# Greketrotny/RayZath

Hardware: AMD Instinct MI355X
Metric: Mrays/s (path segments, primary+secondary) at 1920x1080 depth 8 (higher is better)
Workload: dtype f32; 1 GPU; Cornell box 1920x1080 depth 8; max_depth=8, triangles=16, instances=8, traversal=workgroup-binned, integrator=CPU kernel (parity-checked), pipeline=resident (one kernel per step)

## Files before the change

rayzath_amd/csrc/hiprz_api.hip:

```cpp
#include <hip/hip_runtime.h>

#include <algorithm>
#include <cmath>
#include <cstdio>
#include <cstdlib>
#include <cstring>
#include <string>
#include <vector>

#include "hiprz.h"
#include "hiprz_ctx.hpp"
#include "hiprz_device.hpp"

using namespace hiprz;


__global__ void __launch_bounds__(256) rz_order_keys_kernel(const uint32_t* cost, uint32_t* keys, uint32_t n) {
    const uint32_t i = blockIdx.x * 256u + threadIdx.x;
    if (i < n) keys[i] = 0x00FFFFFFu - (cost[i] < 0x00FFFFFFu ? cost[i] : 0x00FFFFFFu);
}

__global__ void rz_pass_update_kernel(uint32_t* pass) { *pass += 1u; }
__global__ void rz_pass_reset_kernel(uint32_t* pass) { *pass = 0u; }
__global__ void rz_pass_add_kernel(uint32_t* pass, uint32_t n) { *pass += n; }
// ... 93 lines not shown
                if (kind >= 4u) {
                    const bool of_a = kind < 6u;
                    WalkRay probe = q;
                    probe.far_ = RZ_FLT_MAX;
                    float t = 0.0f, u, v, det;
                    if (tri_hit(xyz(of_a ? ta[0] : tb[0]), xyz(of_a ? ta[1] : tb[1]), xyz(of_a ? ta[2] : tb[2]), probe, t, u, v, det)) {
                        if (kind & 1u) q.far_ = t;
                        else q.near_ = t;
                    }
                }
                const bool has_b = (h & 0xC00u) != 0u;
                WalkRay seq = q;
                uint32_t seq_tri = 0xFFFFFFFFu;
                float seq_b1 = 0.0f, seq_b2 = 0.0f;
                bool seq_external = false;
                {
                    float t, u, v, det;
                    if (tri_hit(xyz(ta[0]), xyz(ta[1]), xyz(ta[2]), seq, t, u, v, det)) {
                        seq.far_ = t;
                        seq_tri = 0u, seq_b1 = u, seq_b2 = v, seq_external = det > 0.0f;
                    }
                    if (has_b && tri_hit(xyz(tb[0]), xyz(tb[1]), xyz(tb[2]), seq, t, u, v, det)) {
                        seq.far_ = t;
                        seq_tri = 1u, seq_b1 = u, seq_b2 = v, seq_external = det > 0.0f;
                    }
                }
                LeafBest best;
                best.far_ = q.far_, best.triangle = 0xFFFFFFFFu, best.b1 = best.b2 = 0.0f, best.external = false;
                tri_pair_step(ta[0], ta[1], ta[2], has_b ? tb[0] : ta[0], has_b ? tb[1] : ta[1], has_b ? tb[2] : ta[2], 0u, has_b ? 1u : 0u, has_b, q, best);
                if (__float_as_uint(best.far_) != __float_as_uint(seq.far_) || best.triangle != seq_tri || __float_as_uint(best.b1) != __float_as_uint(seq_b1) ||
                    __float_as_uint(best.b2) != __float_as_uint(seq_b2) || best.external != seq_external)
                    bad += 1;
            }
        }
    }
    atomicAdd(&out[0], (unsigned long long)bad);
    atomicAdd(&out[1], (unsigned long long)tested);
    atomicAdd(&out[2], (unsigned long long)undecided);
}

namespace hiprz {
thread_local std::string g_create_error;
int fail(hiprz_ctx* ctx, int code, const std::string& msg) {
    if (ctx) ctx->error = msg;
    else g_create_error = msg;
    return code;
}
std::vector<KernelEntry>& kernel_table() {
    static std::vector<KernelEntry> table;
    return table;
}
void register_kernel(const void* stub, const char* name) { kernel_table().push_back(KernelEntry{stub, name}); }
int resolve_kernels(int device) {
    static std::vector<int> checked;
    for (int d : checked)
        if (d == device) return HIPRZ_OK;
    for (const KernelEntry& e : kernel_table()) {
        hipFuncAttributes attr;
        const hipError_t err = hipFuncGetAttributes(&attr, e.stub);
        if (err != hipSuccess) {
            (void)hipGetLastError();
            return fail(nullptr, HIPRZ_ERR_DEVICE, std::string("libhiprz.so is inconsistent: the loaded gfx950 code objects do not hold a kernel the host side can launch (") +
                                                       hipGetErrorString(err) + "): " + e.name + " — rebuild (make -C rayzath_amd/csrc; tools/check_kernels.py)");
        }
    }
    checked.push_back(device);
// ... 991 lines not shown
```

rayzath_amd/csrc/hiprz_device.hpp:

```cpp
#pragma once
#include <hip/hip_runtime.h>
#include <stdint.h>

#include "hiprz.h"
#include "hiprz_end.hpp"
#include "hiprz_lds.hpp"
#include "hiprz_shard.hpp"

#define RZ_DEV __device__ __forceinline__
#include "hiprz_flat_pick.hpp"
#include "hiprz_pair_pick.hpp"

namespace hiprz {

#ifndef RZ_FUSED_SHARED_RCP
#define RZ_FUSED_SHARED_RCP 0
#endif
#ifndef RZ_TRACE_SHARED_RCP
#define RZ_TRACE_SHARED_RCP 1
#endif
#ifndef RZ_BATCH_SHARED_RCP
#define RZ_BATCH_SHARED_RCP 1
#endif
#ifndef RZ_FLAT_PACKED_BOXES
#define RZ_FLAT_PACKED_BOXES 0
#endif
#ifndef RZ_FLAT_PAIR_TRIS
#define RZ_FLAT_PAIR_TRIS 1
#endif
#ifndef RZ_TRACE_MIN_WAVES
#define RZ_TRACE_MIN_WAVES 5
#endif
#define RZ_PI_F 3.14159265358979323846f
#define RZ_GUARD_LIMIT (1u << 26)
#ifndef RZ_WALK_GUARD
#define RZ_WALK_GUARD 0
#endif
#if RZ_WALK_GUARD
#define RZ_GUARD(counter) \
    if (++(counter) > RZ_GUARD_LIMIT) break
#else
#define RZ_GUARD(counter) (void)(counter)
#endif
#define RZ_FLT_MAX 3.402823466e+38f

#define RZ_SINF(x) sinf(x)
#define RZ_COSF(x) cosf(x)
#define RZ_SINCOSF(x, s, c) sincosf((x), &(s), &(c))
#define RZ_ACOSF(x) acosf(x)
#define RZ_ASINF(x) asinf(x)
#define RZ_ATAN2F(y, x) atan2f(y, x)
#define RZ_POWF(x, y) powf(x, y)
#define RZ_EXPF(x) expf(x)
#define RZ_LOGF(x) logf(x)

struct DScene {
    const float4* nodes;
    const uint32_t* tlas_order;
    const float4* tris;
    const float4* tri_attrs;
    const float4* instances;
    const int32_t* inst_materials;
    const float4* materials;
    const float4* textures;
    const uint8_t* texels;
    const float4* spot_lights;
    const float4* direct_lights;
    uint32_t n_instances;
    uint32_t tlas_root;
    uint32_t n_spot_lights;
    uint32_t n_direct_lights;
    uint32_t fast_div;
    uint32_t hot_bytes;
    const float4* hot;
    uint32_t off_nodes, off_tlas_order, off_instances, off_tris, off_tri_attrs, off_materials, off_inst_materials;
    uint32_t world_stack_entries;
    uint32_t mesh_stack_entries;
    float bounds_min[3];
    float bounds_scale[3];
    uint32_t top_count;
    const uint32_t* node_skip;
    uint32_t walk_k, walk_l;
    uint32_t walk_advance;
    uint32_t world_advance;
    uint32_t walk_h;
    const float4* nodes64;
    uint32_t shadow_variant;
    const float4* shadow_nodes64;
    const uint32_t* shadow_order;
    uint32_t shadow_root;
    uint32_t sort_variant;
};

RZ_DEV void repoint_hot(DScene& v, const unsigned char* base) {
    v.nodes = reinterpret_cast<const float4*>(base + v.off_nodes);
    v.tlas_order = reinterpret_cast<const uint32_t*>(base + v.off_tlas_order);
    v.instances = reinterpret_cast<const float4*>(base + v.off_instances);
    v.tris = reinterpret_cast<const float4*>(base + v.off_tris);
    v.tri_attrs = reinterpret_cast<const float4*>(base + v.off_tri_attrs);
    v.materials = reinterpret_cast<const float4*>(base + v.off_materials);
    v.inst_materials = reinterpret_cast<const int32_t*>(base + v.off_inst_materials);
}

struct DCamera {
    float position[3];
    float x_axis[3], y_axis[3], z_axis[3];
    uint32_t width, height;
    float tan_half_fov, aspect_ratio;
    float near_, far_;
    float focal_distance, aperture, exposure_time;
};

struct DConfig {
    uint32_t max_depth, spot_samples, direct_samples, seed;
    uint32_t flags;
};

struct DFrame {
    float4* st0;
    float4* st1;
    float2* st2;
    float4* accum;
    float4* hit0;
    uint32_t* hit1;
    float* depth;
    uint32_t* rgba8;
    const uint32_t* pass;
    unsigned long long* counters;
    uint32_t tiles_x;
    uint32_t rank, world;
    uint32_t n_local_tiles;
    uint32_t* sort_key;
    const uint32_t* perm;
    uint32_t xcd_swizzle;
    float4* nee;
// ... 333 lines not shown
    r = __builtin_elementwise_fma(nd, q, n);
    return __builtin_elementwise_fma(r, yy, q);
}
RZ_DEV void box_range_pairs(float4 b0, float4 b1, const WalkRayPairs& p, float& tmin, float& tmax) {
    const f2 tx = div_pairs(f2{b0.x, b0.y} - p.ox, p.ndx, p.yx);
    const f2 ty = div_pairs(f2{b0.z, b0.w} - p.oy, p.ndy, p.yy);
    const f2 tz = div_pairs(f2{b1.x, b1.y} - p.oz, p.ndz, p.yz);
    tmin = vmax3(vmin(tx.x, tx.y), vmin(ty.x, ty.y), vmin(tz.x, tz.y));
    tmax = vmin3(vmax(tx.x, tx.y), vmax(ty.x, ty.y), vmax(tz.x, tz.y));
}
template <bool SHARED_RCP>
RZ_DEV void box_range_packed(float4 b0, float4 b1, const WalkRay& r, float& tmin, float& tmax) {
#if RZ_FLAT_PACKED_BOXES
    if (SHARED_RCP && __all(r.fast)) {
        box_range_pairs(b0, b1, splat_pairs(r), tmin, tmax);
        return;
    }
    box_range_unpacked<false>(b0, b1, r, tmin, tmax);
#else
    box_range_unpacked<SHARED_RCP>(b0, b1, r, tmin, tmax);
#endif
}
template <bool SHARED_RCP>
RZ_DEV bool box_hit_packed(float4 b0, float4 b1, const WalkRay& r) {
    float tmin, tmax;
    box_range_packed<SHARED_RCP>(b0, b1, r, tmin, tmax);
    return !(tmax < r.near_ || tmin > tmax || tmin > r.far_);
}

struct v3p {
    f2 x, y, z;
};
RZ_DEV v3p pair3(float4 a, float4 b) { return v3p{f2{a.x, b.x}, f2{a.y, b.y}, f2{a.z, b.z}}; }
RZ_DEV float det_nudge(float det) { return float(uint32_t(det > -1.0e-7f) & uint32_t(det < 1.0e-7f)) * 1.0e-7f; }
RZ_DEV void tri_hit2(v3p v1, v3p edge1, v3p edge2, const WalkRay& r, bool& inside_a, bool& inside_b, f2& t_out, f2& b1_out, f2& b2_out, f2& det_out) {
    const f2 dx = {r.d.x, r.d.x}, dy = {r.d.y, r.d.y}, dz = {r.d.z, r.d.z};
    const v3p pvec = {dy * edge2.z - dz * edge2.y, dz * edge2.x - dx * edge2.z, dx * edge2.y - dy * edge2.x};
    f2 det = edge1.x * pvec.x + edge1.y * pvec.y + edge1.z * pvec.z;
    det = det + f2{det_nudge(det.x), det_nudge(det.y)};
    const f2 inv_det = {1.0f / det.x, 1.0f / det.y};
    const v3p tvec = {f2{r.o.x, r.o.x} - v1.x, f2{r.o.y, r.o.y} - v1.y, f2{r.o.z, r.o.z} - v1.z};
    const f2 b1 = (tvec.x * pvec.x + tvec.y * pvec.y + tvec.z * pvec.z) * inv_det;
    const v3p qvec = {tvec.y * edge1.z - tvec.z * edge1.y, tvec.z * edge1.x - tvec.x * edge1.z, tvec.x * edge1.y - tvec.y * edge1.x};
    const f2 b2 = (dx * qvec.x + dy * qvec.y + dz * qvec.z) * inv_det;
    const f2 sum = b1 + b2;
    const f2 t = (edge2.x * qvec.x + edge2.y * qvec.y + edge2.z * qvec.z) * inv_det;
    inside_a = !(b1.x < 0.0f || b1.x > 1.0f) && !(b2.x < 0.0f || sum.x > 1.0f) && !(t.x <= r.near_);
    inside_b = !(b1.y < 0.0f || b1.y > 1.0f) && !(b2.y < 0.0f || sum.y > 1.0f) && !(t.y <= r.near_);
    t_out = t, b1_out = b1, b2_out = b2, det_out = det;
}
struct LeafBest {
    float far_;
    uint32_t triangle;
    float b1, b2;
    bool external;
};
RZ_DEV void tri_pair_step(float4 a0, float4 a1, float4 a2, float4 b0, float4 b1, float4 b2, uint32_t ia, uint32_t ib, bool has_b,
                          const WalkRay& r, LeafBest& best) {
    f2 t, u, v, det;
    bool inside_a, inside_b;
    tri_hit2(pair3(a0, b0), pair3(a1, b1), pair3(a2, b2), r, inside_a, inside_b, t, u, v, det);
    const PairPick pick = pair_pick(inside_a, inside_b && has_b, t.x, t.y, best.far_);
    best.far_ = pick.far_;
    if (pick.winner != 0u) {
        const bool second = pick.winner == 2u;
        best.triangle = second ? ib : ia;
        best.b1 = second ? u.y : u.x, best.b2 = second ? v.y : v.x;
        best.external = (second ? det.y : det.x) > 0.0f;
    }
}

struct LdsStack {
    uint32_t* column;
    uint32_t sp;
    RZ_DEV explicit LdsStack(uint32_t* lds_column) : column(lds_column), sp(0) {}
    RZ_DEV uint32_t mark() const { return sp; }
    RZ_DEV uint32_t next(uint32_t base) {
        if (sp == base) return RZ_END;
        sp -= 1;
        return column[sp * blockDim.x];
    }
    RZ_DEV uint32_t descend(uint32_t first_child) {
        column[sp * blockDim.x] = first_child + 1u;
        sp += 1;
        return first_child;
    }
};

template <bool RCP>
RZ_DEV float to_local(const InstanceXform& x, const WalkRay& g, WalkRay& l, bool scene_fast) {
    l.o = transform_backward(x.xa, x.ya, x.za, g.o - x.position);
    l.d = transform_backward(x.xa, x.ya, x.za, g.d);
    if (!x.unit_scale) {
        l.o = l.o / x.scale;
        l.d = l.d / x.scale;
    }
    const float len = magnitude(l.d);
    l.near_ = g.near_ * len;
    l.far_ = g.far_ * len;
// ... 229 lines not shown
            load_instance_box(s, flat_id(fw.ids, k), ib0, ib1);
            float tmin, tmax;
            box_range_unpacked<RZ_FLAT_PACKED_BOXES ? false : RCP>(ib0, ib1, g, tmin, tmax);
            if (counting) { RZ_PHASE(1); RZ_COUNT(box_tests); }
            mask |= uint32_t(!(tmax < g.near_ || tmin > tmax)) << k;
            tm[k] = tmin;
        }
    }
    return mask;
}

template <bool COUNT, bool RCP>
RZ_DEV void binned_visit(const DScene& s, const BinnedLds& lds, uint32_t* mesh_column, bool scene_fast, uint32_t slot, Counters& cnt) {
    RZ_PHASE(2);
    const uint32_t item = lds.items[slot], inst = (item & 0x7FFFFFFFu) >> 8, src = item & 255u;
    WalkRay w;
    w.o = V3(lds.ray[0 * 256 + src], lds.ray[1 * 256 + src], lds.ray[2 * 256 + src]);
    w.d = V3(lds.ray[3 * 256 + src], lds.ray[4 * 256 + src], lds.ray[5 * 256 + src]);
    w.near_ = lds.ray[6 * 256 + src], w.far_ = lds.ray[7 * 256 + src];
    const InstanceXform x = load_instance_xform(s, inst);
    WalkRay lr;
    const float len = to_local<RCP>(x, w, lr, scene_fast);
#if RZ_FLAT_PAIR_TRIS
    const float4 n0 = s.nodes[2 * x.blas_root], n1 = s.nodes[2 * x.blas_root + 1];
    const bool wide = (item & RZ_BIN_WIDE) != 0u;
    if (wide || (__float_as_uint(n1.w) & HIPRZ_NODE_LEAF) != 0u) {
        const uint32_t j = wide ? slot & 7u : 0u, partner = wide ? 8u : 1u;
        RZ_PHASE(3);
        if (j == 0u) { RZ_COUNT(box_tests); }
        LeafBest best;
        best.far_ = lr.far_, best.triangle = 0xFFFFFFFFu, best.b1 = best.b2 = 0.0f, best.external = false;
        if (box_hit_packed<RCP>(n0, n1, lr)) {
            const uint32_t begin = __float_as_uint(n1.z), end = begin + (__float_as_uint(n1.w) & HIPRZ_NODE_COUNT_MASK);
            for (uint32_t i = begin + j; i < end; i += 2u * partner) {
                const bool has_b = i + partner < end;
                const uint32_t ib = has_b ? i + partner : i;
                const float4 a0 = s.tris[3 * i], a1 = s.tris[3 * i + 1], a2 = s.tris[3 * i + 2];
                const float4 b0 = s.tris[3 * ib], b1 = s.tris[3 * ib + 1], b2 = s.tris[3 * ib + 2];
                RZ_PHASE(4);
                if constexpr (COUNT) cnt.tri_tests += has_b ? 2u : 1u;
                tri_pair_step(a0, a1, a2, b0, b1, b2, i, ib, has_b, lr, best);
            }
        }
        bool mine = best.triangle != 0xFFFFFFFFu;
        if (wide) {
            const uint32_t wide_t = mine ? __float_as_uint(best.far_) : 0xFFFFFFFFu;
            const uint32_t t_min = octet_min(wide_t);
            const bool nearest = wide_t != 0xFFFFFFFFu && wide_t == t_min;
            const uint32_t first = octet_min(nearest ? best.triangle : 0xFFFFFFFFu);
            mine = nearest && best.triangle == first;
        }
        if (mine) {
            lds.ray[6 * 256 + src] = lr.near_ / len;
            lds.ray[7 * 256 + src] = best.far_ / len;
            lds.hit[0 * 256 + src] = best.triangle;
            lds.hit[1 * 256 + src] = best.external ? 1u : 0u;
            lds.hit[2 * 256 + src] = __float_as_uint(best.b1);
            lds.hit[3 * 256 + src] = __float_as_uint(best.b2);
            lds.hit[4 * 256 + src] = inst;
        }
        return;
    }
#endif
    if (item & RZ_BIN_WIDE) {
        const uint32_t j = slot & 7u;
        const float4 n0 = s.nodes[2 * x.blas_root], n1 = s.nodes[2 * x.blas_root + 1];
        RZ_PHASE(3);
        if (j == 0u) { RZ_COUNT(box_tests); }
        uint32_t wide_t = 0xFFFFFFFFu, wide_tri = 0xFFFFFFFFu;
        float wide_b1 = 0.0f, wide_b2 = 0.0f;
        bool wide_external = false;
        const float visit_near = lr.near_;
        if (box_hit_packed<RCP>(n0, n1, lr)) {
            const uint32_t begin = __float_as_uint(n1.z), end = begin + (__float_as_uint(n1.w) & HIPRZ_NODE_COUNT_MASK);
            for (uint32_t i = begin + j; i < end; i += 8u) {
// ... 1634 lines not shown
```

rayzath_amd/csrc/hiprz_end.hpp:

```cpp
#pragma once
#define RZ_END 0xFFFFFFFFu
```

rayzath_amd/csrc/hiprz_scene.hip:

```cpp
#include <hip/hip_runtime.h>

#include <algorithm>
#include <cstdio>
#include <cstdlib>
#include <cstring>
#include <string>
#include <vector>

#include "hiprz.h"
#include "hiprz_ctx.hpp"
#include "hiprz_device.hpp"
#include "hiprz_scene_host.hpp"

using namespace hiprz;

#define RZ_FANOUT_OTHER_DEVICES(c, call)                                                                                       \
    for (hiprz_ctx* p : (c)->peers) {                                                                                         \
        if (p->device == (c)->device) continue;                                                                               \
        const int rz_rc = (call);                                                                                             \
        if (rz_rc != HIPRZ_OK) return fail(c, rz_rc, "device " + std::to_string(p->device) + ": " + p->error);              \
    }

namespace {

// ... 38 lines not shown
}
int restart_after_geometry_change(hiprz_ctx* c) {
    c->reset_pending = true;
    stale_guides(c);
    for (auto& f : c->parked) f.reset_pending = true;
    return HIPRZ_OK;
}
bool validate_device_trees() { return !std::getenv("HIPRZ_TRUST_DEVICE_TREES"); }
uint32_t env_u32(const char* name, uint32_t otherwise) {
    const char* v = std::getenv(name);
    return v ? uint32_t(std::atoi(v)) : otherwise;
}
uint32_t sort_variant_for(const hiprz_ctx* c, uint32_t n_lights) { return n_lights && c->shadow_sort == 0 ? 0u : 4u; }

int build_shadow_world_tree(hiprz_ctx* c, const std::vector<hiprz_instance>& dinst, DScene& d) {
    d.shadow_nodes64 = nullptr, d.shadow_order = nullptr, d.shadow_root = RZ_END;
    const std::vector<uint32_t>& members = c->world_members;
    if (!c->shadow_tree || members.empty() || members.size() > 160u) return HIPRZ_OK;
    std::vector<uint32_t> rec, order;
    build_shadow_tree(dinst, members, rec, order);
    (void)hipSetDevice(c->device);
    RZ_HIP(c, c->shadow_nodes64.resize(rec.size()));
    RZ_HIP(c, c->shadow_order.resize(order.size()));
    RZ_HIP(c, hipStreamSynchronize(c->stream));
    RZ_HIP(c, hipMemcpy(c->shadow_nodes64.ptr, rec.data(), rec.size() * sizeof(uint32_t), hipMemcpyHostToDevice));
    RZ_HIP(c, hipMemcpy(c->shadow_order.ptr, order.data(), order.size() * sizeof(uint32_t), hipMemcpyHostToDevice));
    d.shadow_nodes64 = reinterpret_cast<const float4*>(c->shadow_nodes64.ptr), d.shadow_order = c->shadow_order.ptr, d.shadow_root = 0u;
    return HIPRZ_OK;
}


int copy_scene(hiprz_ctx* c, const hiprz_scene& sc, const PackedScene& packed, bool device_trees) {
    (void)hipSetDevice(c->device);
    RZ_HIP(c, c->hot.assign(packed.blob.data(), packed.blob.size(), c->stream));
    RZ_HIP(c, c->node_skip.assign(packed.skip.data(), packed.skip.size(), c->stream));
    if (device_trees) {
        hiprz_node unused{};
        unused.meta = HIPRZ_NODE_LEAF;
        std::vector<hiprz_node> all(packed.node_capacity, unused);
        std::copy(packed.nodes.begin(), packed.nodes.end(), all.begin());
        RZ_HIP(c, c->dev_nodes.assign(reinterpret_cast<const uint8_t*>(all.data()), all.size() * sizeof(hiprz_node), c->stream));
        RZ_HIP(c, hipStreamSynchronize(c->stream));
    }
    RZ_HIP(c, c->nodes64.assign(packed.nodes64.data(), packed.nodes64.size(), c->stream));
    RZ_HIP(c, c->textures.assign(sc.textures, sc.n_textures, c->stream));
    RZ_HIP(c, c->texels.assign(sc.texels, sc.texel_bytes, c->stream));
    RZ_HIP(c, c->spot_lights.assign(sc.spot_lights, sc.n_spot_lights, c->stream));
    RZ_HIP(c, c->direct_lights.assign(sc.direct_lights, sc.n_direct_lights, c->stream));
    RZ_HIP(c, hipStreamSynchronize(c->stream));
    return HIPRZ_OK;
}

void bind_tunables(hiprz_ctx* c, DScene& d, uint32_t n_lights) {
    d.walk_k = env_u32("HIPRZ_WALK_K", 4u), d.walk_l = env_u32("HIPRZ_WALK_L", 8u);
    d.walk_h = env_u32("HIPRZ_WALK_H", 65u);
    d.sort_variant = env_u32("HIPRZ_SORT_KEY", sort_variant_for(c, n_lights));
    d.shadow_variant = env_u32("HIPRZ_SHADOW_KEY", 0x500u);
    d.walk_advance = env_u32("HIPRZ_WALK_ADVANCE", 1u);
    d.world_advance = env_u32("HIPRZ_WORLD_ADVANCE", 8u);
}

void bind_scene(hiprz_ctx* c, const ChosenTrees& trees, const PackedScene& packed, const SceneCheck& chk) {
    const hiprz_scene& sc = trees.scene;
    DScene& d = c->dscene;
    c->stack_entries = chk.world_depth + chk.mesh_depth + 2u;
    d.world_stack_entries = chk.world_depth + 1u;
    d.mesh_stack_entries = chk.mesh_depth + 1u;
    d.off_nodes = packed.off_nodes, d.off_tlas_order = packed.off_tlas_order, d.off_instances = packed.off_instances, d.off_tris = packed.off_tris;
    d.off_tri_attrs = packed.off_tri_attrs, d.off_materials = packed.off_materials, d.off_inst_materials = packed.off_inst_materials;
    d.hot_bytes = uint32_t(packed.blob.size());
    d.hot = reinterpret_cast<const float4*>(c->hot.ptr);
    d.nodes = reinterpret_cast<const float4*>(trees.device_trees() ? c->dev_nodes.ptr : c->hot.ptr + d.off_nodes);
    d.tlas_order = reinterpret_cast<const uint32_t*>(c->hot.ptr + d.off_tlas_order);
    d.instances = reinterpret_cast<const float4*>(c->hot.ptr + d.off_instances);
    d.tris = reinterpret_cast<const float4*>(c->hot.ptr + d.off_tris);
    d.tri_attrs = reinterpret_cast<const float4*>(c->hot.ptr + d.off_tri_attrs);
    d.materials = reinterpret_cast<const float4*>(c->hot.ptr + d.off_materials);
    d.inst_materials = reinterpret_cast<const int32_t*>(c->hot.ptr + d.off_inst_materials);
    d.fast_div = packed.fast_div ? 1u : 0u;
    d.textures = reinterpret_cast<const float4*>(c->textures.ptr);
    d.texels = c->texels.ptr;
    d.spot_lights = reinterpret_cast<const float4*>(c->spot_lights.ptr);
    d.direct_lights = reinterpret_cast<const float4*>(c->direct_lights.ptr);
    d.n_instances = sc.n_instances;
    d.tlas_root = packed.tlas_root;
    d.node_skip = c->node_skip.ptr;
    std::memcpy(d.bounds_min, packed.bounds_min, 12), std::memcpy(d.bounds_scale, packed.bounds_scale, 12);
    d.top_count = std::min<uint32_t>(uint32_t(packed.nodes.size()), kTopCacheNodes);
    d.nodes64 = reinterpret_cast<const float4*>(c->nodes64.ptr);
    d.n_spot_lights = sc.n_spot_lights;
    d.n_direct_lights = sc.n_direct_lights;
    bind_tunables(c, d, sc.n_spot_lights + sc.n_direct_lights);
    c->n_nodes = sc.n_nodes;
    c->flat_world = packed.flat_world;
    c->n_textures = sc.n_textures;
    c->lds_scene = size_t(d.hot_bytes) + size_t(c->stack_entries) * 1024u + BinnedLds::kFixedBytes <= kLdsSceneLimit;
    c->scene_tree = trees.tree;
    if (trees.own_trees) c->lds_scene = false;
    c->n_tris = sc.n_tris, c->n_tlas_order = sc.n_tlas_order;
    c->device_meshes.clear(), c->instance_mesh.clear();
    c->world_members = packed.world_members;
}

// ... 195 lines not shown
```

rayzath_amd/csrc/hiprz_scene_host.cpp:

```cpp
#include "hiprz_scene_host.hpp"

#include <algorithm>

namespace hiprz {

namespace {
struct TreeCheck {
    const hiprz_scene* sc;
    std::vector<uint32_t>& skip;
    std::vector<uint8_t> visited;
    uint32_t max_depth = 0;
    std::string error;
    std::vector<uint32_t> world_leaves;

    bool walk(uint32_t root, bool is_world) {
        struct Item {
            uint32_t node, skip, depth;
        };
        std::vector<Item> stack{{root, RZ_END, 1u}};
        while (!stack.empty()) {
            const Item it = stack.back();
            stack.pop_back();
            if (it.node >= sc->n_nodes) return err("node index out of range");
            if (visited[it.node]) return err("node reachable twice (trees must be disjoint and acyclic)");
// ... 207 lines not shown
    const uint32_t max_nodes = sc->n_nodes + 2u * sc->n_tris + sc->n_instances + 1u;
    std::vector<uint32_t> order(sc->n_tris), roots(sc->n_instances ? sc->n_instances : 1u);
    uint32_t n_nodes = 0u, tlas_root = 0u;
    out.nodes.resize(max_nodes);
    if (hiprz_rebuild_mesh_trees(sc, tree, out.nodes.data(), max_nodes, &n_nodes, order.data(), roots.data(), &tlas_root) != HIPRZ_OK) {
        if (tree_mode == HIPRZ_TREE_AUTO) return HIPRZ_OK;
        error = "upload_scene: the mesh trees could not be rebuilt (leaves of a mesh must tile one range of triangles)";
        return HIPRZ_ERR_INVALID;
    }
    out.nodes.resize(n_nodes);
    out.identity_order = true;
    for (uint32_t i = 0; i < sc->n_tris && out.identity_order; ++i) out.identity_order = order[i] == i;
    if (!out.identity_order) {
        out.tris.resize(sc->n_tris), out.attrs.resize(sc->n_tris);
        for (uint32_t i = 0; i < sc->n_tris; ++i) {
            out.tris[i] = sc->tris[order[i]];
            out.tris[i].pad0 = order[i];
            out.attrs[i] = sc->tri_attrs[order[i]];
        }
        out.scene.tris = out.tris.data(), out.scene.tri_attrs = out.attrs.data();
    }
    out.instances.assign(sc->instances, sc->instances + sc->n_instances);
    for (uint32_t i = 0; i < sc->n_instances; ++i) out.instances[i].blas_root = roots[i];
    out.scene.n_nodes = n_nodes, out.scene.nodes = out.nodes.data(), out.scene.tlas_root = tlas_root;
    out.scene.instances = out.instances.data();
    out.tree = tree, out.own_trees = true;
    if (check_scene(&out.scene, chk) != HIPRZ_OK) {
        error = "upload_scene: rebuilt trees: " + chk.error;
        return HIPRZ_ERR_INVALID;
    }
    return HIPRZ_OK;
}

int pack_scene(const ChosenTrees& trees, DerivedTables&& derived, PackedScene& out, std::string& error) {
    const hiprz_scene* sc = &trees.scene;
    out.new_index = std::move(derived.new_index), out.nodes = std::move(derived.dnodes), out.skip = std::move(derived.dskip);
    const std::vector<uint32_t>& new_index = out.new_index;
    std::vector<hiprz_node>& dnodes = out.nodes;
    out.fast_div = true;
    for (const auto& n : dnodes)
        for (int a = 0; a < 3; ++a) out.fast_div = out.fast_div && coord_ok(n.bb_min[a]) && coord_ok(n.bb_max[a]);
    for (uint32_t i = 0; i < sc->n_instances; ++i)
        for (int a = 0; a < 3; ++a) out.fast_div = out.fast_div && coord_ok(sc->instances[i].bb_min[a]) && coord_ok(sc->instances[i].bb_max[a]);
    for (auto& n : dnodes) interleave_box(n);
    out.instances.assign(sc->instances, sc->instances + sc->n_instances);
    for (uint32_t i = 0; i < sc->n_instances; ++i) {
        hiprz_instance& in = out.instances[i];
        if (in.blas_root < sc->n_nodes) in.blas_root = new_index[in.blas_root];
        pack_instance_placement(in, sc->instances[i]);
    }
    std::vector<uint8_t>& blob = out.blob;
    blob.clear();
    auto append = [&blob](const void* src, size_t bytes) {
        const uint32_t off = uint32_t(blob.size());
        blob.resize(blob.size() + ((bytes + 15u) & ~size_t(15)), 0);
        if (bytes) std::memcpy(blob.data() + off, src, bytes);
        return off;
    };
    out.off_nodes = append(dnodes.data(), sizeof(hiprz_node) * dnodes.size());
    out.off_tlas_order = append(sc->tlas_order, sizeof(uint32_t) * sc->n_tlas_order);
    out.off_instances = append(out.instances.data(), sizeof(hiprz_instance) * out.instances.size());
    {
        std::vector<hiprz_tri> dtris(sc->tris, sc->tris + sc->n_tris);
        std::vector<hiprz_tri_attr> dattrs(sc->tri_attrs, sc->tri_attrs + sc->n_tris);
        for (uint32_t i = 0; i < sc->n_tris; ++i) {
            hiprz_tri& t = dtris[i];
            hiprz_tri_attr& a = dattrs[i];
// ... 25 lines not shown
            if (root >= sc->n_nodes) continue;
            if (mesh_of_root[root] == RZ_END) {
                const hiprz_node& leaf = sc->nodes[root];
                DeviceMesh m;
                m.tri_first = leaf.begin, m.n_tris = leaf.meta & HIPRZ_NODE_COUNT_MASK;
                m.ref_first = m.n_tris ? (trees.identity_order ? leaf.begin : sc->tris[leaf.begin].pad0) : 0u;
                m.leaf_slot = new_index[root];
                std::memcpy(m.bb_min, leaf.bb_min, 12), std::memcpy(m.bb_max, leaf.bb_max, 12);
                mesh_of_root[root] = uint32_t(out.device_meshes.size());
                out.device_meshes.push_back(m);
            }
            out.instance_mesh[i] = mesh_of_root[root];
        }
        uint32_t cursor = uint32_t(dnodes.size());
        if (!(cursor & 1u)) cursor += 1u;
        out.world_region = cursor;
        cursor += 2u * sc->n_instances + 1u;
        out.node_capacity = device_build_regions(out.device_meshes, cursor);
        out.skip.resize(out.node_capacity, RZ_END);
    }
    out.nodes64.assign(size_t(out.node_capacity ? out.node_capacity : 1) * 16u, RZ_END);
    for (size_t n = 0; n < dnodes.size(); ++n) {
        std::memcpy(&out.nodes64[n * 16u], &dnodes[n], sizeof(hiprz_node));
        std::memcpy(&out.nodes64[n * 16u + 8u], &derived.dskip8[n * 8u], 32);
    }

    out.tlas_root = sc->n_instances ? new_index[sc->tlas_root] : 0u;
    for (int a = 0; a < 3; ++a) {
        const float lo = sc->n_instances ? sc->nodes[sc->tlas_root].bb_min[a] : 0.0f, hi = sc->n_instances ? sc->nodes[sc->tlas_root].bb_max[a] : 0.0f;
        out.bounds_min[a] = lo;
        out.bounds_scale[a] = hi > lo ? 32.0f / (hi - lo) : 0.0f;
    }
    out.flat_world = sc->n_instances != 0u && (sc->nodes[sc->tlas_root].meta & HIPRZ_NODE_LEAF) && (sc->nodes[sc->tlas_root].meta & HIPRZ_NODE_COUNT_MASK) <= 8u;
    std::vector<uint8_t> member(sc->n_instances ? sc->n_instances : 1u, 0);
    for (uint32_t k = 0; k < sc->n_tlas_order; ++k)
        if (sc->tlas_order[k] < sc->n_instances) member[sc->tlas_order[k]] = 1;
    out.world_members.clear();
    for (uint32_t i = 0; i < sc->n_instances; ++i)
        if (member[i]) out.world_members.push_back(i);
    return HIPRZ_OK;
}

uint32_t enter_device_roots(std::vector<hiprz_instance>& instances, const std::vector<uint32_t>& instance_mesh, const std::vector<DeviceMesh>& meshes,
                            uint32_t world_slots) {
    for (size_t i = 0; i < instances.size(); ++i)
        if (instance_mesh[i] != RZ_END && meshes[instance_mesh[i]].region != RZ_END) instances[i].blas_root = meshes[instance_mesh[i]].region;
    uint32_t emitted = world_slots;
    for (const auto& m : meshes) emitted += m.n_slots;
    return emitted;
}

void build_shadow_tree(const std::vector<hiprz_instance>& dinst, const std::vector<uint32_t>& members, std::vector<uint32_t>& rec,
                       std::vector<uint32_t>& order) {
    auto box_of = [&](uint32_t i) { return packed_instance_box(dinst[i]); };
    auto grow = [](InstanceBox& b, const InstanceBox& o) {
        for (int a = 0; a < 3; ++a) b.mn[a] = std::min(b.mn[a], o.mn[a]), b.mx[a] = std::max(b.mx[a], o.mx[a]);
    };
    auto area = [](const InstanceBox& b) {
        const float x = b.mx[0] - b.mn[0], y = b.mx[1] - b.mn[1], z = b.mx[2] - b.mn[2];
        return x * y + y * z + z * x;
    };
    const uint32_t n = uint32_t(members.size());
    order = members, rec.assign(size_t(2u * n) * 16u, RZ_END);
    std::vector<uint32_t> sorted, best;
    std::vector<float> left_area;
    struct Task {
// ... 49 lines not shown
```

rayzath_amd/csrc/hiprz_scene_host.hpp:

```cpp
#pragma once
#include <cstdint>
#include <cstring>
#include <string>
#include <vector>

#include "hiprz.h"
#include "hiprz_end.hpp"

namespace hiprz {

constexpr uint32_t kLeafMax = 4u;

struct DeviceMesh {
    uint32_t tri_first = 0, n_tris = 0;
    uint32_t ref_first = 0;
    uint32_t region = 0xFFFFFFFFu;
    uint32_t leaf_slot = 0xFFFFFFFFu;
    uint32_t n_slots = 0;
    float bb_min[3] = {0, 0, 0}, bb_max[3] = {0, 0, 0};
};
uint32_t device_build_regions(std::vector<DeviceMesh>& meshes, uint32_t first_free_slot);

inline bool coord_ok(float x) {
    uint32_t b;
    std::memcpy(&b, &x, 4);
    const uint32_t e = (b >> 23) & 0xFFu;
    return (b & 0x7FFFFFFFu) == 0u || (e >= 127u - 60u && e < 127u + 40u);
}
inline void interleave_box(hiprz_node& n) {
    const float v[6] = {n.bb_min[0], n.bb_max[0], n.bb_min[1], n.bb_max[1], n.bb_min[2], n.bb_max[2]};
    std::memcpy(n.bb_min, v, 12), std::memcpy(n.bb_max, v + 3, 12);
}
inline void deinterleave_box(hiprz_node& n) {
    const float v[6] = {n.bb_min[0], n.bb_min[1], n.bb_min[2], n.bb_max[0], n.bb_max[1], n.bb_max[2]};
    n.bb_min[0] = v[0], n.bb_max[0] = v[1], n.bb_min[1] = v[2], n.bb_max[1] = v[3], n.bb_min[2] = v[4], n.bb_max[2] = v[5];
}
inline void pack_instance_placement(hiprz_instance& d, const hiprz_instance& in) {
    const float v[6] = {in.bb_min[0], in.bb_max[0], in.bb_min[1], in.bb_max[1], in.bb_min[2], in.bb_max[2]};
    const uint32_t unit = (in.scale[0] == 1.0f && in.scale[1] == 1.0f && in.scale[2] == 1.0f) ? 1u : 0u;
    std::memcpy(d.position, in.position, 12), std::memcpy(d.scale, in.scale, 12);
    std::memcpy(d.x_axis, in.x_axis, 12), std::memcpy(d.y_axis, in.y_axis, 12), std::memcpy(d.z_axis, in.z_axis, 12);
    d.pad0 = unit;
    d.bb_min[0] = v[0], d.bb_min[1] = v[1], d.bb_min[2] = v[2];
    std::memcpy(&d.pad2, &v[3], 4);
// ... 25 lines not shown
    std::vector<uint32_t> dskip8;
};
int derive_tables(const hiprz_scene* sc, SceneCheck& chk, DerivedTables& out);

struct ChosenTrees {
    hiprz_scene scene{};
    uint32_t tree = HIPRZ_TREE_REFERENCE;
    bool own_trees = false;
    bool identity_order = false;
    std::vector<hiprz_node> nodes;
    std::vector<hiprz_tri> tris;
    std::vector<hiprz_tri_attr> attrs;
    std::vector<hiprz_instance> instances;
    ChosenTrees() = default;
    ChosenTrees(const ChosenTrees&) = delete;
    ChosenTrees& operator=(const ChosenTrees&) = delete;
    bool device_trees() const { return own_trees && tree == HIPRZ_TREE_DEVICE; }
};
int choose_trees(const hiprz_scene* sc, uint32_t tree_mode, size_t lds_limit, SceneCheck& chk, ChosenTrees& out, std::string& error);

struct PackedScene {
    std::vector<uint8_t> blob;
    uint32_t off_nodes = 0, off_tlas_order = 0, off_instances = 0, off_tris = 0, off_tri_attrs = 0, off_materials = 0, off_inst_materials = 0;
    std::vector<uint32_t> new_index;
    std::vector<hiprz_node> nodes;
    std::vector<uint32_t> skip;
    std::vector<uint32_t> nodes64;
    std::vector<hiprz_instance> instances;
    std::vector<uint32_t> world_members;
    bool fast_div = true;
    float bounds_min[3] = {0, 0, 0}, bounds_scale[3] = {0, 0, 0};
    uint32_t tlas_root = 0;
    bool flat_world = false;
    std::vector<DeviceMesh> device_meshes;
    std::vector<uint32_t> instance_mesh;
    uint32_t world_region = 0, node_capacity = 0;
};
int pack_scene(const ChosenTrees& trees, DerivedTables&& derived, PackedScene& out, std::string& error);

uint32_t enter_device_roots(std::vector<hiprz_instance>& instances, const std::vector<uint32_t>& instance_mesh, const std::vector<DeviceMesh>& meshes,
                            uint32_t world_slots);

void build_shadow_tree(const std::vector<hiprz_instance>& instances, const std::vector<uint32_t>& members, std::vector<uint32_t>& records,
                       std::vector<uint32_t>& order);

}
```

Baseline: 12080 Mrays/s.

## Pre-pack triangle pairs into interleaved records for flat-world leaf traversal

Adds a host-built pair section to the hot scene blob. It holds a per-instance offset table and 72-byte records that interleave two triangles' data component-wise, so the flat-world leaf loop can load ready-made paired operands instead of gathering and shuffling two triangles. The leaf loop now strides over pairs rather than over partner-spaced triangles. A packed reciprocal helper (rcp_pair) and a bit-exact self-test are also added, but that reciprocal path is off by default. The cost is extra host packing and a blocking stream sync at upload, plus a more complex device indexing path that relies on the pair section being present.

```diff
diff --git a/rayzath_amd/csrc/hiprz_api.hip b/rayzath_amd/csrc/hiprz_api.hip
--- a/rayzath_amd/csrc/hiprz_api.hip
+++ b/rayzath_amd/csrc/hiprz_api.hip
@@ -149,6 +149,26 @@
                     __float_as_uint(best.b2) != __float_as_uint(seq_b2) || best.external != seq_external)
                     bad += 1;
             }
+            {
+                auto operand = [&](uint32_t k) {
+                    const uint32_t w = mix32(h + 0x51EDu * k), sel = (w >> 3) & 7u, sign = w & 0x80000000u, frac = mix32(w) & 0x7FFFFFu;
+                    if (sel == 0u) return __uint_as_float(mix32(w ^ 0x3C6EF372u));
+                    if (sel == 1u) return unit(50u + k) * 2.0e-7f;
+                    if (sel == 2u) return __uint_as_float(sign | __float_as_uint(1.0e-7f + (unit(52u + k) - 0.5f) * 1.0e-9f));
+                    if (sel == 3u) return __uint_as_float(sign | ((253u + (w >> 8) % 2u) << 23) | frac);
+                    if (sel == 4u) return __uint_as_float(sign | (((w >> 8) % 3u) << 23) | frac);
+                    if (sel == 5u) {
+                        const uint32_t special[4] = {0x00000000u, 0x7F800000u, 0x7FC00000u | frac, 0x7F800001u};
+                        return __uint_as_float(sign | special[(w >> 8) & 3u]);
+                    }
+                    return __uint_as_float(sign | ((64u + (w >> 8) % 128u) << 23) | frac);
+                };
+                const f2 x = {operand(1u), operand(2u)};
+                const f2 got = rcp_pair(x);
+                const float want_x = 1.0f / x.x, want_y = 1.0f / x.y;
+                if (__float_as_uint(got.x) != __float_as_uint(want_x) && !(got.x != got.x && want_x != want_x)) bad += 1;
+                if (__float_as_uint(got.y) != __float_as_uint(want_y) && !(got.y != got.y && want_y != want_y)) bad += 1;
+            }
         }
     }
     atomicAdd(&out[0], (unsigned long long)bad);
diff --git a/rayzath_amd/csrc/hiprz_device.hpp b/rayzath_amd/csrc/hiprz_device.hpp
--- a/rayzath_amd/csrc/hiprz_device.hpp
+++ b/rayzath_amd/csrc/hiprz_device.hpp
@@ -27,6 +27,12 @@
 #endif
 #ifndef RZ_FLAT_PAIR_TRIS
 #define RZ_FLAT_PAIR_TRIS 1
+#endif
+#ifndef RZ_FLAT_PAIR_RECORDS
+#define RZ_FLAT_PAIR_RECORDS 1
+#endif
+#ifndef RZ_FLAT_PK_DIV
+#define RZ_FLAT_PK_DIV 0
 #endif
 #ifndef RZ_TRACE_MIN_WAVES
 #define RZ_TRACE_MIN_WAVES 5
@@ -84,6 +90,7 @@
     uint32_t walk_advance;
     uint32_t world_advance;
     uint32_t walk_h;
+    uint32_t off_pairs;
     const float4* nodes64;
     uint32_t shadow_variant;
     const float4* shadow_nodes64;
@@ -101,6 +108,9 @@
     v.materials = reinterpret_cast<const float4*>(base + v.off_materials);
     v.inst_materials = reinterpret_cast<const int32_t*>(base + v.off_inst_materials);
 }
+
+static_assert(sizeof(DScene) == 256, "off_pairs fills a padding word: the kernels' argument layout is what it was");
+RZ_DEV const unsigned char* pair_section(const DScene& s) { return reinterpret_cast<const unsigned char*>(s.nodes) - s.off_nodes + s.off_pairs; }
 
 struct DCamera {
     float position[3];
@@ -500,13 +510,32 @@
     f2 x, y, z;
 };
 RZ_DEV v3p pair3(float4 a, float4 b) { return v3p{f2{a.x, b.x}, f2{a.y, b.y}, f2{a.z, b.z}}; }
+RZ_DEV f2 rcp_pair(f2 x) {
+    bool scaled_x, scaled_y, unused;
+    const f2 den = {__builtin_amdgcn_div_scalef(1.0f, x.x, false, &unused), __builtin_amdgcn_div_scalef(1.0f, x.y, false, &unused)};
+    const f2 num = {__builtin_amdgcn_div_scalef(1.0f, x.x, true, &scaled_x), __builtin_amdgcn_div_scalef(1.0f, x.y, true, &scaled_y)};
+    const f2 rcp = {__builtin_amdgcn_rcpf(den.x), __builtin_amdgcn_rcpf(den.y)};
+    const f2 nden = -den, one = {1.0f, 1.0f};
+    const f2 e0 = __builtin_elementwise_fma(nden, rcp, one);
+    const f2 r1 = __builtin_elementwise_fma(e0, rcp, rcp);
+    const f2 q0 = num * r1;
+    const f2 e1 = __builtin_elementwise_fma(nden, q0, num);
+    const f2 q1 = __builtin_elementwise_fma(e1, r1, q0);
+    const f2 e2 = __builtin_elementwise_fma(nden, q1, num);
+    return f2{__builtin_amdgcn_div_fixupf(__builtin_amdgcn_div_fmasf(e2.x, r1.x, q1.x, scaled_x), x.x, 1.0f),
+              __builtin_amdgcn_div_fixupf(__builtin_amdgcn_div_fmasf(e2.y, r1.y, q1.y, scaled_y), x.y, 1.0f)};
+}
 RZ_DEV float det_nudge(float det) { return float(uint32_t(det > -1.0e-7f) & uint32_t(det < 1.0e-7f)) * 1.0e-7f; }
 RZ_DEV void tri_hit2(v3p v1, v3p edge1, v3p edge2, const WalkRay& r, bool& inside_a, bool& inside_b, f2& t_out, f2& b1_out, f2& b2_out, f2& det_out) {
     const f2 dx = {r.d.x, r.d.x}, dy = {r.d.y, r.d.y}, dz = {r.d.z, r.d.z};
     const v3p pvec = {dy * edge2.z - dz * edge2.y, dz * edge2.x - dx * edge2.z, dx * edge2.y - dy * edge2.x};
     f2 det = edge1.x * pvec.x + edge1.y * pvec.y + edge1.z * pvec.z;
     det = det + f2{det_nudge(det.x), det_nudge(det.y)};
+#if RZ_FLAT_PK_DIV
+    const f2 inv_det = rcp_pair(det);
+#else
     const f2 inv_det = {1.0f / det.x, 1.0f / det.y};
+#endif
     const v3p tvec = {f2{r.o.x, r.o.x} - v1.x, f2{r.o.y, r.o.y} - v1.y, f2{r.o.z, r.o.z} - v1.z};
     const f2 b1 = (tvec.x * pvec.x + tvec.y * pvec.y + tvec.z * pvec.z) * inv_det;
     const v3p qvec = {tvec.y * edge1.z - tvec.z * edge1.y, tvec.z * edge1.x - tvec.x * edge1.z, tvec.x * edge1.y - tvec.y * edge1.x};
@@ -533,6 +562,19 @@
     if (pick.winner != 0u) {
         const bool second = pick.winner == 2u;
         best.triangle = second ? ib : ia;
+        best.b1 = second ? u.y : u.x, best.b2 = second ? v.y : v.x;
+        best.external = (second ? det.y : det.x) > 0.0f;
+    }
+}
+RZ_DEV void tri_pair_step(v3p v1, v3p edge1, v3p edge2, uint32_t ia, bool has_b, const WalkRay& r, LeafBest& best) {
+    f2 t, u, v, det;
+    bool inside_a, inside_b;
+    tri_hit2(v1, edge1, edge2, r, inside_a, inside_b, t, u, v, det);
+    const PairPick pick = pair_pick(inside_a, inside_b && has_b, t.x, t.y, best.far_);
+    best.far_ = pick.far_;
+    if (pick.winner != 0u) {
+        const bool second = pick.winner == 2u;
+        best.triangle = second ? ia + 1u : ia;
         best.b1 = second ? u.y : u.x, best.b2 = second ? v.y : v.x;
         best.external = (second ? det.y : det.x) > 0.0f;
     }
@@ -828,6 +870,22 @@
         best.far_ = lr.far_, best.triangle = 0xFFFFFFFFu, best.b1 = best.b2 = 0.0f, best.external = false;
         if (box_hit_packed<RCP>(n0, n1, lr)) {
             const uint32_t begin = __float_as_uint(n1.z), end = begin + (__float_as_uint(n1.w) & HIPRZ_NODE_COUNT_MASK);
+#if RZ_FLAT_PAIR_RECORDS
+            const uint32_t count = end - begin, n_pairs = (count + 1u) >> 1;
+            const unsigned char* section = pair_section(s);
+            const float2* rec = reinterpret_cast<const float2*>(section + 8u * reinterpret_cast<const uint16_t*>(section)[inst]);
+            for (uint32_t p = j; p < n_pairs; p += wide ? 8u : 1u) {
+                const float2* q = rec + p * (RZ_PAIR_RECORD_BYTES / 8u);
+                const float2 v1x = q[0], v1y = q[1], v1z = q[2], e1x = q[3], e1y = q[4], e1z = q[5], e2x = q[6], e2y = q[7], e2z = q[8];
+                const bool has_b = 2u * p + 1u < count;
+                const uint32_t i = begin + 2u * p;
+                RZ_PHASE(4);
+                if constexpr (COUNT) cnt.tri_tests += has_b ? 2u : 1u;
+                tri_pair_step(v3p{f2{v1x.x, v1x.y}, f2{v1y.x, v1y.y}, f2{v1z.x, v1z.y}}, v3p{f2{e1x.x, e1x.y}, f2{e1y.x, e1y.y}, f2{e1z.x, e1z.y}},
+                              v3p{f2{e2x.x, e2x.y}, f2{e2y.x, e2y.y}, f2{e2z.x, e2z.y}}, i, has_b, lr, best);
+            }
+            (void)partner;
+#else
             for (uint32_t i = begin + j; i < end; i += 2u * partner) {
                 const bool has_b = i + partner < end;
                 const uint32_t ib = has_b ? i + partner : i;
@@ -837,6 +895,7 @@
                 if constexpr (COUNT) cnt.tri_tests += has_b ? 2u : 1u;
                 tri_pair_step(a0, a1, a2, b0, b1, b2, i, ib, has_b, lr, best);
             }
+#endif
         }
         bool mine = best.triangle != 0xFFFFFFFFu;
         if (wide) {
diff --git a/rayzath_amd/csrc/hiprz_end.hpp b/rayzath_amd/csrc/hiprz_end.hpp
--- a/rayzath_amd/csrc/hiprz_end.hpp
+++ b/rayzath_amd/csrc/hiprz_end.hpp
@@ -1,2 +1,3 @@
 #pragma once
 #define RZ_END 0xFFFFFFFFu
+#define RZ_PAIR_RECORD_BYTES 72u
diff --git a/rayzath_amd/csrc/hiprz_scene.hip b/rayzath_amd/csrc/hiprz_scene.hip
--- a/rayzath_amd/csrc/hiprz_scene.hip
+++ b/rayzath_amd/csrc/hiprz_scene.hip
@@ -94,7 +94,14 @@
 
 int copy_scene(hiprz_ctx* c, const hiprz_scene& sc, const PackedScene& packed, bool device_trees) {
     (void)hipSetDevice(c->device);
-    RZ_HIP(c, c->hot.assign(packed.blob.data(), packed.blob.size(), c->stream));
+    if (packed.pair_section.empty()) {
+        RZ_HIP(c, c->hot.assign(packed.blob.data(), packed.blob.size(), c->stream));
+    } else {
+        std::vector<uint8_t> hot(packed.blob);
+        hot.insert(hot.end(), packed.pair_section.begin(), packed.pair_section.end());
+        RZ_HIP(c, c->hot.assign(hot.data(), hot.size(), c->stream));
+        RZ_HIP(c, hipStreamSynchronize(c->stream));
+    }
     RZ_HIP(c, c->node_skip.assign(packed.skip.data(), packed.skip.size(), c->stream));
     if (device_trees) {
         hiprz_node unused{};
@@ -130,7 +137,8 @@
     d.mesh_stack_entries = chk.mesh_depth + 1u;
     d.off_nodes = packed.off_nodes, d.off_tlas_order = packed.off_tlas_order, d.off_instances = packed.off_instances, d.off_tris = packed.off_tris;
     d.off_tri_attrs = packed.off_tri_attrs, d.off_materials = packed.off_materials, d.off_inst_materials = packed.off_inst_materials;
-    d.hot_bytes = uint32_t(packed.blob.size());
+    d.off_pairs = uint32_t(packed.blob.size());
+    d.hot_bytes = uint32_t(packed.hot_bytes());
     d.hot = reinterpret_cast<const float4*>(c->hot.ptr);
     d.nodes = reinterpret_cast<const float4*>(trees.device_trees() ? c->dev_nodes.ptr : c->hot.ptr + d.off_nodes);
     d.tlas_order = reinterpret_cast<const uint32_t*>(c->hot.ptr + d.off_tlas_order);
diff --git a/rayzath_amd/csrc/hiprz_scene_host.cpp b/rayzath_amd/csrc/hiprz_scene_host.cpp
--- a/rayzath_amd/csrc/hiprz_scene_host.cpp
+++ b/rayzath_amd/csrc/hiprz_scene_host.cpp
@@ -263,7 +263,7 @@
     return HIPRZ_OK;
 }
 
-int pack_scene(const ChosenTrees& trees, DerivedTables&& derived, PackedScene& out, std::string& error) {
+int pack_scene(const ChosenTrees& trees, DerivedTables&& derived, PackedScene& out, std::string& error, bool pair_records) {
     const hiprz_scene* sc = &trees.scene;
     out.new_index = std::move(derived.new_index), out.nodes = std::move(derived.dnodes), out.skip = std::move(derived.dskip);
     const std::vector<uint32_t>& new_index = out.new_index;
@@ -355,6 +355,44 @@
         out.bounds_scale[a] = hi > lo ? 32.0f / (hi - lo) : 0.0f;
     }
     out.flat_world = sc->n_instances != 0u && (sc->nodes[sc->tlas_root].meta & HIPRZ_NODE_LEAF) && (sc->nodes[sc->tlas_root].meta & HIPRZ_NODE_COUNT_MASK) <= 8u;
+    out.pair_section.clear();
+    if (pair_records && out.flat_world && !trees.own_trees) {
+        const uint32_t table_bytes = ((sc->n_instances + 3u) & ~3u) * 2u;
+        std::vector<uint16_t> table(table_bytes / 2u, kPairNone);
+        std::vector<uint32_t> first_of_root(sc->n_nodes, RZ_END);
+        std::vector<uint8_t> records;
+        bool any = false;
+        for (uint32_t i = 0; i < sc->n_instances; ++i) {
+            const uint32_t root = sc->instances[i].blas_root;
+            if (root >= sc->n_nodes || !(sc->nodes[root].meta & HIPRZ_NODE_LEAF)) continue;
+            if (first_of_root[root] == RZ_END) {
+                first_of_root[root] = (table_bytes + uint32_t(records.size())) / 8u;
+                const uint32_t begin = sc->nodes[root].begin, n = sc->nodes[root].meta & HIPRZ_NODE_COUNT_MASK;
+                for (uint32_t p = 0; 2u * p < n && records.size() < kPairSectionLimit; ++p) {
+                    hiprz_tri ab[2];
+                    std::memcpy(&ab[0], blob.data() + out.off_tris + sizeof(hiprz_tri) * (begin + 2u * p), sizeof(hiprz_tri));
+                    ab[1] = ab[0];
+                    if (2u * p + 1u < n) std::memcpy(&ab[1], blob.data() + out.off_tris + sizeof(hiprz_tri) * (begin + 2u * p + 1u), sizeof(hiprz_tri));
+                    float rec[kPairRecordBytes / 4u];
+                    for (int k = 0; k < 3; ++k)
+                        for (int e = 0; e < 2; ++e) rec[2 * k + e] = ab[e].v1[k], rec[6 + 2 * k + e] = ab[e].v2[k], rec[12 + 2 * k + e] = ab[e].v3[k];
+                    const size_t at = records.size();
+                    records.resize(at + kPairRecordBytes);
+                    std::memcpy(records.data() + at, rec, kPairRecordBytes);
+                }
+            }
+            table[i] = uint16_t(first_of_root[root]), any = true;
+        }
+        if (any && table_bytes + records.size() <= kPairSectionLimit) {
+            out.pair_section.assign((table_bytes + records.size() + 15u) & ~size_t(15), 0);
+            std::memcpy(out.pair_section.data(), table.data(), table_bytes);
+            if (!records.empty()) std::memcpy(out.pair_section.data() + table_bytes, records.data(), records.size());
+        }
+        if (out.hot_bytes() > 0xFFFFFFF0ull) {
+            error = "scene geometry exceeds 4 GiB";
+            return HIPRZ_ERR_INVALID;
+        }
+    }
     std::vector<uint8_t> member(sc->n_instances ? sc->n_instances : 1u, 0);
     for (uint32_t k = 0; k < sc->n_tlas_order; ++k)
         if (sc->tlas_order[k] < sc->n_instances) member[sc->tlas_order[k]] = 1;
diff --git a/rayzath_amd/csrc/hiprz_scene_host.hpp b/rayzath_amd/csrc/hiprz_scene_host.hpp
--- a/rayzath_amd/csrc/hiprz_scene_host.hpp
+++ b/rayzath_amd/csrc/hiprz_scene_host.hpp
@@ -10,6 +10,9 @@
 namespace hiprz {
 
 constexpr uint32_t kLeafMax = 4u;
+constexpr uint32_t kPairRecordBytes = RZ_PAIR_RECORD_BYTES;
+constexpr uint16_t kPairNone = 0xFFFFu;
+constexpr size_t kPairSectionLimit = 8u * 0xFFFEu;
 
 struct DeviceMesh {
     uint32_t tri_first = 0, n_tris = 0;
@@ -101,11 +104,13 @@
     float bounds_min[3] = {0, 0, 0}, bounds_scale[3] = {0, 0, 0};
     uint32_t tlas_root = 0;
     bool flat_world = false;
+    std::vector<uint8_t> pair_section;
+    size_t hot_bytes() const { return blob.size() + pair_section.size(); }
     std::vector<DeviceMesh> device_meshes;
     std::vector<uint32_t> instance_mesh;
     uint32_t world_region = 0, node_capacity = 0;
 };
-int pack_scene(const ChosenTrees& trees, DerivedTables&& derived, PackedScene& out, std::string& error);
+int pack_scene(const ChosenTrees& trees, DerivedTables&& derived, PackedScene& out, std::string& error, bool pair_records = true);
 
 uint32_t enter_device_roots(std::vector<hiprz_instance>& instances, const std::vector<uint32_t>& instance_mesh, const std::vector<DeviceMesh>& meshes,
                             uint32_t world_slots);
```

Result: faster. 12420 Mrays/s (median of 6 runs) (+2.9%).
